# nubot-nudt/LCR-Net

Hardware: AMD Instinct MI355X
Metric: scans/s (120k-pt KITTI-shape scan -> 256-D descriptor) (higher is better)
Workload: dtype f32 (K-deep GEMMs, K >= 288 and N >= 64: fp32 operands as bf16 x 3 split, 6 of 9 products on the bf16 matrix cores, fp32 accumulate — error vs fp64 <= the fp32-MFMA kernel's; every other GEMM, KPConv and attention: fp32 MFMA); 1 GPU; configs[1]: batch of 8 synthetic 64-beam scans (~120k pts, 0.3 m voxel -> ~16k pts), voxelise + 3 subsamples + 10 radius searches + KPConv encoder + NetVLAD, seeded random weights; distinct_input_batches=4, streams=pre-processing stream (own host thread, 2 batches ahead) + 2 encoder stream(s), parallelism=scan-parallel x1, all-gather of descriptors

## Files before the change

include/lcr_hip_debug.h:

```cpp
#ifndef LCR_HIP_DEBUG_H
#define LCR_HIP_DEBUG_H

#ifdef __cplusplus
extern "C" {
#endif

void lcr_gemm_debug_force_tile(int tile);
void lcr_gemm_debug_deep(int mode);
void lcr_gemm_debug_streamk(int mode);
void lcr_groupnorm_debug_general(int on);
void lcr_kpconv_debug_off64(int on);

#ifdef __cplusplus
}
#endif
#endif
```

lcr-net_amd/_lib.py:

```python
import ctypes
import os
import re
import types

import torch

_PKG = os.path.dirname(os.path.abspath(__file__))
LIB_PATH = os.path.join(_PKG, "liblcr_hip.so")

_lib = None

HEADERS = [os.path.join(_PKG, "..", "include", h) for h in ("lcr_hip.h", "lcr_hip_debug.h")]
_SCALARS = {"int": ctypes.c_int, "int64_t": ctypes.c_int64, "uint32_t": ctypes.c_uint32, "uint64_t": ctypes.c_uint64, "unsigned": ctypes.c_uint,
            "size_t": ctypes.c_size_t, "float": ctypes.c_float, "double": ctypes.c_double}
_RESULTS = {"int": ctypes.c_int, "void": None, "const char*": ctypes.c_char_p}


def parse_header(text):
    text = re.sub(r"/\*.*?\*/|//[^\n]*", " ", text, flags=re.S)
    text = re.sub(r"^\s*#.*$", "", text, flags=re.M)
    sigs = {}
    for m in re.finditer(r"\b(lcr_\w+)\s*\(", text):
        name = m.group(1)
        head = text[:m.start()]
        res = re.sub(r"\s*\*", "*", " ".join(head[max(head.rfind(c) for c in ";{}") + 1:].split()))
        tail = re.match(r"([^()]*)\)\s*;", text[m.end():])
        if res not in _RESULTS or tail is None:
            raise RuntimeError("%s: cannot parse its prototype (result type %r)" % (name, res))
        args = []
        for p in ([] if tail.group(1).strip() in ("", "void") else tail.group(1).split(",")):
            words = re.sub(r"\bconst\b", " ", p).split()
            ctype = ctypes.c_void_p if "*" in p else _SCALARS.get(" ".join(words[:-1] if len(words) > 1 else words))
            if ctype is None:
                raise RuntimeError("%s: parameter %r has no ctypes mapping" % (name, " ".join(p.split())))
            args.append(ctype)
        sigs[name] = (_RESULTS[res], args)
    return sigs


_RELEASES_GIL = {"lcr_roformer_forward", "lcr_precompute_batch", "lcr_precompute_batch_rows", "lcr_precompute_batch_rows_ex", "lcr_hashmap_bucket_host", "lcr_encoder_forward", "lcr_encoder_forward_ex", "lcr_ktimer_read",
                 "lcr_ktimer_read2", "lcr_hashmap_order_host", "lcr_ransac_sample_host", "lcr_icp_point_to_point", "lcr_icp_point_to_plane", "lcr_netvlad_forward", "lcr_log_sinkhorn", "lcr_log_sinkhorn_ex",
                 "lcr_local_global_registration", "lcr_local_global_registration_ex", "lcr_retrieval_topk", "lcr_stream_spin"}


def build():
    import importlib.util
    spec = importlib.util.spec_from_file_location("_lcr_build", os.path.join(_PKG, "csrc", "build.py"))
    mod = importlib.util.module_from_spec(spec)
    spec.loader.exec_module(mod)
    return mod.build()


_RETURNS_VALUE = {"lcr_version", "lcr_kpconv_mask_ok", "lcr_gemm_split_ok", "lcr_ktimer_read", "lcr_ktimer_read2"}


def __getattr__(name):
    if name == "call":
        lib()
        return call
    raise AttributeError(name)


def _raise_on_rc(rc, fn, args):
    if rc:
        check(rc, fn.__name__)
    return rc


def lib():
    global _lib, call
    if _lib is None:
        if not os.path.exists(LIB_PATH):
            raise RuntimeError(
                "liblcr_hip.so not found at %s — build it with `python lcr-net_amd/csrc/build.py` "
                "(there is no CPU fallback for the lcr-net_amd hot path)" % LIB_PATH)
        sigs = {}
        for header in HEADERS:
            with open(header) as f:
                sigs.update(parse_header(f.read()))
        L = ctypes.CDLL(LIB_PATH)
        K = ctypes.PyDLL(LIB_PATH) if os.environ.get("LCR_CTYPES_KEEP_GIL", "1") != "0" else L
        checked = types.SimpleNamespace()
        for name, (res, args) in sigs.items():
            if not hasattr(L, name):
                continue
            dll = L if name in _RELEASES_GIL else K
            for view, fn in ((L, getattr(dll, name)), (checked, dll[name])):
                fn.restype, fn.argtypes = res, args
                if view is checked and res is ctypes.c_int and name not in _RETURNS_VALUE:
                    fn.errcheck = _raise_on_rc
                setattr(view, name, fn)
        _lib, call = L, checked
    return _lib


def check(rc, what):
    if rc != 0:
        msg = lib().lcr_last_error()
        raise RuntimeError("%s failed (rc=%d): %s" % (what, rc, msg.decode() if msg else ""))


def ptr(t):
    return ctypes.c_void_p(t.data_ptr()) if t is not None else ctypes.c_void_p(0)


def stream_ptr(device=None):
    idx = device.index if isinstance(device, torch.device) else None
    if idx is None:
        idx = torch.cuda.current_device() if not isinstance(device, int) else device
    return ctypes.c_void_p(torch._C._cuda_getCurrentRawStream(idx))


def require_cuda(*tensors):
    for t in tensors:
        if t is not None and not t.is_cuda:
            raise RuntimeError("lcr-net_amd ops run on the GPU only: got a %s tensor (no CPU fallback)" % t.device)


def workspace(nbytes, device):
    return torch.empty(max(int(nbytes), 256), dtype=torch.uint8, device=device)


def ws_size(name, *args):
    lib()
    n = ctypes.c_size_t(0)
    getattr(call, name)(*args, ctypes.byref(n))
    return n.value


def ws(name, *args, device):
    return workspace(ws_size(name, *args), device)
```

lcr-net_amd/csrc/gemm.h:

```cpp
#pragma once
#include <cstdlib>

#include "common.h"

namespace lcr {

typedef float floatx16 __attribute__((ext_vector_type(16)));

constexpr int GM_BK = 32;
constexpr int GM_T = 256;

constexpr int GM_MAX_BATCH = 64;
struct GemmBatch {
  int     count;
  int     strided;
  int     k[GM_MAX_BATCH];
  int64_t a_off[GM_MAX_BATCH], b_off[GM_MAX_BATCH], c_off[GM_MAX_BATCH];
};

struct GemmEpilogue {
  const float*   bias;
  const float*   rowdiv;
  const int64_t* seg_len;
  int            S;
  int            groups;
  double*        stats;
};

struct ANorm {
  const double* stats;
  const float*  gamma;
  const float*  beta;
  int           groups;
  float         eps, slope;
};
constexpr int AN_KMAX = 256;

__device__ __forceinline__ float4 ld4(const float* p) { return *reinterpret_cast<const float4*>(p); }

__device__ __forceinline__ void anorm_load_affine(const ANorm& an, int K, float (&an_g)[2], float (&an_b)[2]) {
#pragma unroll
  for (int u = 0; u < 2; ++u) {
    const int e = threadIdx.x + u * GM_T;
    an_g[u] = an_b[u] = 0.f;
    if (e < 2 * K) {
      const int k = e >= K ? e - K : e;
      an_g[u] = an.gamma[k];
      an_b[u] = an.beta[k];
    }
  }
}

__device__ __forceinline__ void anorm_build_table(const ANorm& an, const GemmEpilogue& ep, int K, int blk_first, const float (&an_g)[2],
                                                  const float (&an_b)[2], float* __restrict__ s_an) {
  const int gs = K / an.groups;
  __shared__ float2 s_mr[2 * 64];
  for (int e = threadIdx.x; e < 2 * an.groups; e += GM_T) {
    const int slot = e >= an.groups ? 1 : 0, g = e - slot * an.groups;
    const int sg = min(blk_first + slot, ep.S - 1);
    const double cnt = static_cast<double>(ep.seg_len[sg]) * gs;
    double sx = 0.0, sxx = 0.0;
    for (int rep = 0; rep < GN_REPLICAS; ++rep) {
      const int64_t o = ((static_cast<int64_t>(rep) * ep.S + sg) * an.groups + g) * 2;
      sx += an.stats[o];
      sxx += an.stats[o + 1];
    }
    const double mean = sx / cnt;
    const double var = fmax(sxx / cnt - mean * mean, 0.0);
    s_mr[e] = make_float2(static_cast<float>(mean), static_cast<float>(1.0 / sqrt(var + static_cast<double>(an.eps))));
  }
  __syncthreads();
#pragma unroll
  for (int u = 0; u < 2; ++u) {
    const int e = threadIdx.x + u * GM_T;
    if (e < 2 * K) {
      const int slot = e >= K ? 1 : 0, k = e - slot * K;
      const float2 mr = s_mr[slot * an.groups + k / gs];
      const float sc = mr.y * an_g[u];
      s_an[slot * 2 * AN_KMAX + k] = sc;
      s_an[slot * 2 * AN_KMAX + AN_KMAX + k] = fmaf(-mr.x, sc, an_b[u]);
    }
  }
  __syncthreads();
}

template <int BM, int BN, int WM, int WN, int NT>
__device__ __forceinline__ void gemm_epilogue(floatx16 (&acc)[NT], float* __restrict__ C, int64_t M, int N, int64_t m0, int n0, int64_t m_tile,
                                              const GemmEpilogue& ep, const float (&bias_v)[NT], int blk_first, int64_t blk_seg_start,
                                              int64_t blk_seg_end, int wm, int wn, int lane) {
  const bool want_stats = ep.stats != nullptr;
  const int gs = want_stats ? N / ep.groups : 1;
  const int64_t wrow0 = m0 + wm * 32;

  const bool interior = m0 + BM <= M && n0 + BN <= N && M * static_cast<int64_t>(N) < (int64_t(1) << 30);
  if (interior) {
    const unsigned row_l = static_cast<unsigned>(wrow0) + 4u * static_cast<unsigned>(lane >> 5);
#pragma unroll
    for (int j = 0; j < NT; ++j) {
      const unsigned col = static_cast<unsigned>(n0 + wn * (32 * NT) + j * 32 + (lane & 31));
      const float bv = bias_v[j];
      const unsigned off0 = row_l * static_cast<unsigned>(N) + col;
      if (ep.rowdiv) {
#pragma unroll
        for (int r = 0; r < 16; ++r) {
          const unsigned dr = static_cast<unsigned>((r & 3) + 8 * (r >> 2));
          const float v = acc[j][r] / ep.rowdiv[row_l + dr] + bv;
          C[off0 + dr * static_cast<unsigned>(N)] = v;
          acc[j][r] = v;
        }
      } else {
#pragma unroll
        for (int r = 0; r < 16; ++r) {
          const unsigned dr = static_cast<unsigned>((r & 3) + 8 * (r >> 2));
          const float v = acc[j][r] + bv;
          C[off0 + dr * static_cast<unsigned>(N)] = v;
          acc[j][r] = v;
        }
      }
    }
  } else
#pragma unroll
  for (int j = 0; j < NT; ++j) {
    const int col = n0 + wn * (32 * NT) + j * 32 + (lane & 31);
    const float bv = bias_v[j];
#pragma unroll
    for (int r = 0; r < 16; ++r) {
      const int64_t row = wrow0 + (r & 3) + 8 * (r >> 2) + 4 * (lane >> 5);
      float v = acc[j][r];
      if (row < M) {
        if (ep.rowdiv) v = v / ep.rowdiv[row];
        v += bv;
        if (col < N) C[row * N + col] = v;
      } else {
        v = 0.f;
      }
      acc[j][r] = v;
    }
  }

  if (want_stats) {
    __shared__ float s_part[2][2 * WM][BN];
    double* rep = ep.stats + static_cast<int64_t>(m_tile % GN_REPLICAS) * ep.S * ep.groups * 2;
    int64_t seg_start = blk_seg_start, seg_end = blk_seg_end;
    const int64_t blk_last_row = min(m0 + BM - 1, M - 1);
    constexpr int GN_EXACT_ROWS = 32;
    auto exact_segment = [&](int64_t rows) { return rows < GN_EXACT_ROWS && gs <= 32; };
    const bool uniform = blk_last_row < seg_end && !exact_segment(seg_end - seg_start);
    if (uniform) {
#pragma unroll
      for (int j = 0; j < NT; ++j) {
        float s = 0.f, ss = 0.f;
#pragma unroll
        for (int r = 0; r < 16; ++r) {
          s += acc[j][r];
          ss = fmaf(acc[j][r], acc[j][r], ss);
        }
        const int cl = wn * (32 * NT) + j * 32 + (lane & 31);
        s_part[0][2 * wm + (lane >> 5)][cl] = s;
        s_part[1][2 * wm + (lane >> 5)][cl] = ss;
      }
      __syncthreads();
      if (threadIdx.x < BN) {
        const int cl = threadIdx.x;
// ... 98 lines not shown
```

lcr-net_amd/csrc/gemm_f32.hip:

```cpp
#include <cstdio>
#include <map>
#include <mutex>
#include <type_traits>

#include "gemm.h"

namespace lcr {

template <int R, int LD, bool VEC, bool RM = false>
struct LoaderT {
  static constexpr int PIECES = R * 8 / GM_T;
  float4 reg[PIECES];
  unsigned okmask;
  int kb;
  __device__ __forceinline__ void load(const float* __restrict__ src, int64_t rows_total, int K, int64_t r0, int k0) {
    kb = k0;
#pragma unroll
    for (int j = 0; j < PIECES; ++j) {
      const int f = threadIdx.x + GM_T * j;
      const int row = f >> 3, c4 = f & 7;
      int64_t gr = r0 + row;
      gr = gr < rows_total ? gr : rows_total - 1;
      const int gk = k0 + c4 * 4;
      if (VEC) {
// ... 527 lines not shown
static int sk_cu_count() {
  static const int n = [] {
    int dev = 0, cus = 0;
    hipGetDevice(&dev);
    if (hipDeviceGetAttribute(&cus, hipDeviceAttributeMultiprocessorCount, dev) != hipSuccess || cus <= 0) cus = 256;
    return cus;
  }();
  return n;
}

static bool sk_worth(int64_t M, int N, int K) {
  const int cus = sk_cu_count();
  const int64_t tiles = static_cast<int64_t>(div_up(M, 64)) * div_up(N, 64);
  if (K < 480 || tiles < cus / 2 || tiles > 6 * static_cast<int64_t>(cus) || tiles > SK_MAX_TILES) return false;
  const double avg = static_cast<double>(tiles) / cus;
  const double worst = static_cast<double>((tiles + cus - 1) / cus);
  return worst / avg >= 1.10;
}

static int launch_gemm_sk(const float* A, const float* B, float* C, int64_t M, int N, int K, const GemmEpilogue& ep, hipStream_t st) {
  const int cus = sk_cu_count();
  const int64_t iters = static_cast<int64_t>(div_up(M, 64)) * div_up(N, 64) * div_up(K, GM_BK);
  int per_cu = 3;
  while (per_cu > 1 && iters / (static_cast<int64_t>(cus) * per_cu) < 24) --per_cu;
  per_cu = env_int("LCR_SK_PER_CU", per_cu);
  int U = cus * per_cu / 8;
  if (U < 1) U = 1;
  if (8 * U > SK_MAX_GRID) U = SK_MAX_GRID / 8;
  int dev = 0;
  hipGetDevice(&dev);
  GemmStreamK sk;
  {
    std::lock_guard<std::mutex> lk(g_sk_mu);
    SkScratch& sc = g_sk_scratch[{dev, st}];
    if (!sc.partial) {
      if (hipMalloc(reinterpret_cast<void**>(&sc.partial), sizeof(float) * 2 * 16 * GM_T * SK_MAX_GRID) != hipSuccess ||
          hipMalloc(reinterpret_cast<void**>(&sc.arrived), sizeof(uint32_t) * SK_MAX_TILES) != hipSuccess) {
        set_error("lcr_gemm_f32: cannot allocate the stream-K scratch");
        return LCR_EHIP;
      }
      hipMemsetAsync(sc.arrived, 0, sizeof(uint32_t) * SK_MAX_TILES, st);
    }
    sk.partial = sc.partial;
    sk.arrived = sc.arrived;
    sk.U = U;
  }
  LCR_LAUNCH_TIMED((k_gemm_f32_sk<64, 64, 2, 2>), dim3(8 * U), dim3(GM_T), 0, st, A, B, C, M, N, K, ep, sk);
  return check_launch("lcr_gemm_f32");
}

}

using namespace lcr;

static int g_force_tile = 0;
extern "C" void lcr_gemm_debug_force_tile(int t) { g_force_tile = t; }
static int g_force_streamk = -1;
static int g_force_deep = -1;
extern "C" void lcr_gemm_debug_deep(int mode) { g_force_deep = mode; }
extern "C" void lcr_gemm_debug_streamk(int mode) { g_force_streamk = mode; }

enum GemmForm { GF_SCALAR, GF_FORCED_TILE, GF_SHORT, GF_DEEP, GF_STREAMK, GF_TILE };
static GemmForm gemm_form(int64_t M, int N, int K, int transA, int transB, bool vec) {
  static const bool no_short = getenv("LCR_GEMM_NO_SHORT") != nullptr;
  static const int short_k = env_int("LCR_GEMM_SHORT_K", 256);
  static const int deep_env = env_int("LCR_GEMM_DEEP", 1);
  static const int sk_env = env_int("LCR_GEMM_STREAMK", 0);
  if (!vec) return GF_SCALAR;
  if (g_force_tile >= 1 && g_force_tile <= 5) return GF_FORCED_TILE;
  const int deep_mode = g_force_deep >= 0 ? g_force_deep : deep_env;
  const bool deep_ok = !transA && transB && K % GM_BK == 0 && !g_force_tile && M * K < (int64_t(1) << 30) && static_cast<int64_t>(N) * K < (int64_t(1) << 30);
  if (deep_mode == 2 && deep_ok) return GF_DEEP;
  if (!no_short && K <= short_k && !transA) return GF_SHORT;
  if (deep_mode && deep_ok) return GF_DEEP;
  if (N <= 32) return GF_TILE;
  const int sk_mode = g_force_streamk >= 0 ? g_force_streamk : sk_env;
  const bool sk_legal = !transA && !transB && K >= 64 && static_cast<int64_t>(div_up(M, 64)) * div_up(N, 64) <= SK_MAX_TILES;
  if (sk_mode && sk_legal && (sk_mode == 2 || sk_worth(M, N, K))) return GF_STREAMK;
  return GF_TILE;
}

static bool gemm_split_light(int N, int K) {
  switch (K) {
    case 128: return N == 64 || N == 256 || N == 512;
    case 256: return N == 64 || N == 128 || N == 512 || N == 1024;
    default: return false;
  }
}
extern "C" int lcr_gemm_split_ok(int N, int K) {
  static const bool light = env_int("LCR_GEMM_SPLIT_LIGHT", 1) != 0;
  if (N < 64 || K < GM_BK || K % GM_BK != 0) return 0;
  return K >= 288 || (light && K <= AN_KMAX && gemm_split_light(N, K));
}

extern "C" int lcr_gemm_f32_anorm(const float* A, const float* B, float* C, int64_t M, int N, int K, const float* bias,
                                  const double* a_stats, const float* a_gamma, const float* a_beta, int a_groups, float a_eps,
                                  float a_slope, const int64_t* seg_len, int S, int groups, double* stats, void* stream) {
  if (!A || !B || !C || M < 0 || N <= 32 || K <= 0 || K > AN_KMAX || K % 4 != 0 || !a_stats || !a_gamma || !a_beta || a_groups < 1 ||
      K % a_groups != 0 || a_groups > 64 || !seg_len || S < 1 || reinterpret_cast<uintptr_t>(A) % 16 != 0 || reinterpret_cast<uintptr_t>(B) % 16 != 0) {
    set_error("lcr_gemm_f32_anorm: needs 32 < N, K <= 256, K % 4 == 0, a_groups dividing K, a segment table and 16-byte aligned operands");
    return LCR_EARG;
  }
  if (!gemm_stats_ok("lcr_gemm_f32_anorm", stats, seg_len, S, groups, N)) return LCR_EARG;
  hipStream_t st = static_cast<hipStream_t>(stream);
  KernelTimerScope timed(KT_GEMM, st, M, N, K);
  if (M == 0) return LCR_OK;
  GemmEpilogue ep{bias, nullptr, seg_len, S, groups, stats};
  ANorm an{a_stats, a_gamma, a_beta, a_groups, a_eps, a_slope};
  LCR_LAUNCH_TIMED((k_gemm_f32<64, 64, 2, 2, false, true, true, true, true>), dim3(gemm_grid(M, N, 64, 64)), dim3(GM_T), 0, st, A, B, C, M,
                     N, K, ep, GemmBatch{}, an);
  return check_launch("lcr_gemm_f32_anorm");
}

extern "C" int lcr_gemm_f32(const float* A, const float* B, float* C, int64_t M, int N, int K, int transA, int transB, const float* bias,
                            const float* rowdiv, const int64_t* seg_len, int S, int groups, double* stats, void* stream) {
  if (!A || !B || !C || M < 0 || N <= 0 || K <= 0) {
    set_error("lcr_gemm_f32: bad argument");
    return LCR_EARG;
  }
  if (!gemm_stats_ok("lcr_gemm_f32", stats, seg_len, S, groups, N)) return LCR_EARG;
  hipStream_t st = static_cast<hipStream_t>(stream);
  KernelTimerScope timed(KT_GEMM, st, M, N, K);
  if (M == 0) return LCR_OK;
  GemmEpilogue ep{bias, rowdiv, seg_len, S, groups, stats};
  const int64_t lda = transA ? M : K, ldb = transB ? K : N;
  const bool vec = (lda % 4 == 0) && (ldb % 4 == 0) && (reinterpret_cast<uintptr_t>(A) % 16 == 0) && (reinterpret_cast<uintptr_t>(B) % 16 == 0);
  switch (gemm_form(M, N, K, transA, transB, vec)) {
    case GF_SCALAR: return launch_gemm<128, 64, 4, 1, false>(A, B, C, M, N, K, transA, transB, ep, st);
    case GF_FORCED_TILE:
      switch (g_force_tile) {
        case 1: return launch_gemm<128, 128, 4, 1, true>(A, B, C, M, N, K, transA, transB, ep, st);
        case 2: return launch_gemm<128, 64, 4, 1, true>(A, B, C, M, N, K, transA, transB, ep, st);
        case 3: return launch_gemm<128, 32, 4, 1, true>(A, B, C, M, N, K, transA, transB, ep, st);
        case 4: return launch_gemm<64, 64, 2, 2, true>(A, B, C, M, N, K, transA, transB, ep, st);
        default: return launch_gemm<64, 128, 2, 2, true>(A, B, C, M, N, K, transA, transB, ep, st);
      }
    case GF_SHORT:
      if (N <= 32) return launch_gemm<128, 32, 4, 1, true, true>(A, B, C, M, N, K, transA, transB, ep, st);
      return launch_gemm<64, 64, 2, 2, true, true>(A, B, C, M, N, K, transA, transB, ep, st);
    case GF_DEEP: return gemm_deep_launch(A, B, C, M, N, K, ep, st, nullptr, 0);
    case GF_STREAMK: return launch_gemm_sk(A, B, C, M, N, K, ep, st);
    case GF_TILE: break;
  }
  if (N <= 32) return launch_gemm<128, 32, 4, 1, true>(A, B, C, M, N, K, transA, transB, ep, st);
  const int64_t b128 = (M + 127) / 128, nb128 = (N + 127) / 128;
  if (K >= 512 && b128 * nb128 >= 512) return launch_gemm<128, 128, 4, 1, true>(A, B, C, M, N, K, transA, transB, ep, st);
  return launch_gemm<64, 64, 2, 2, true>(A, B, C, M, N, K, transA, transB, ep, st);
}

extern "C" int lcr_kpconv_mask_ok(int64_t M, int N, int K, int split) {
  static const bool off = env_int("LCR_KP_MASK", 1) == 0;
  if (off || M <= 0 || N <= 0 || K % 15 != 0 || mask_kshift(K, K / 15) < 0) return 0;
  if (split) return M * static_cast<int64_t>(K) < (int64_t(1) << 29);
  return gemm_form(M, N, K, 0, 1, true) == GF_DEEP;
}

extern "C" int lcr_gemm_f32_batched_ta(const float* A, const float* B, float* C, int64_t M, int N, int count, const int* k_host,
                                       const int64_t* a_off_host, const int64_t* b_off_host, const int64_t* c_off_host, void* stream) {
  if (!A || !B || !C || M <= 0 || N <= 0 || count < 1 || count > GM_MAX_BATCH || !k_host || !a_off_host || !b_off_host || !c_off_host) {
    set_error("lcr_gemm_f32_batched_ta: bad argument (count <= %d)", GM_MAX_BATCH);
    return LCR_EARG;
  }
  GemmBatch bt = {};
  bt.count = count;
  for (int i = 0; i < count; ++i) {
    bt.k[i] = k_host[i];
// ... 42 lines not shown
```

lcr-net_amd/csrc/gemm_split.hip:

```cpp
#include <type_traits>

#include "gemm.h"

namespace lcr {

typedef __bf16 bf16x8_t __attribute__((ext_vector_type(8)));
typedef __bf16 bf16x2_t __attribute__((ext_vector_type(2)));
typedef float f32x2_t __attribute__((ext_vector_type(2)));
typedef float f32x4_t __attribute__((ext_vector_type(4)));
typedef uint32_t u32x4_t __attribute__((ext_vector_type(4)));

__device__ __forceinline__ uint32_t pk_bf16(float a, float b) {
  f32x2_t v = {a, b};
  return __builtin_bit_cast(uint32_t, __builtin_convertvector(v, bf16x2_t));
}
__device__ __forceinline__ void split2(float x0, float x1, uint32_t& h1, uint32_t& h2, uint32_t& h3) {
  h1 = pk_bf16(x0, x1);
  const float r0 = fsub(x0, __uint_as_float(h1 << 16)), r1 = fsub(x1, __uint_as_float(h1 & 0xffff0000u));
  h2 = pk_bf16(r0, r1);
  const float s0 = fsub(r0, __uint_as_float(h2 << 16)), s1 = fsub(r1, __uint_as_float(h2 & 0xffff0000u));
  h3 = pk_bf16(s0, s1);
}

__global__ __launch_bounds__(256) void k_split_bf16x3(const float* __restrict__ w, int64_t n, uint16_t* __restrict__ planes) {
// ... 137 lines not shown
  if constexpr (ANORM) anorm_load_affine(an, K, an_g, an_b);
  int blk_first = 0;
  int64_t blk_seg_start = 0, blk_seg_end = 0;
  if (ep.stats != nullptr || ANORM) {
    blk_seg_end = ep.seg_len[0];
    while (blk_first + 1 < ep.S && m0 >= blk_seg_end) {
      ++blk_first;
      blk_seg_start = blk_seg_end;
      blk_seg_end += ep.seg_len[blk_first];
    }
  }
  if constexpr (ANORM) {
    const int an_split = static_cast<int>(min(static_cast<int64_t>(BM), blk_seg_end - m0));
#pragma unroll
    for (int j = 0; j < 2; ++j) toff[j] = (srow + j * (T / 8) >= an_split ? 2 * AN_KMAX : 0) + spc * 4;
    anorm_build_table(an, ep, K, blk_first, an_g, an_b, s_an);
  }
  park(I0{}, 0, 0);
  fetch_a(I0{}, 2);
  fetch_b(I1{}, 1);
  __syncthreads();
  auto step = [&](auto lds_c, int t) {
    constexpr int P = decltype(lds_c)::value;
    using NX = std::integral_constant<int, P ^ 1>;
    const char* la = sA + P * STGA + fa;
    bf16x8_t a[4][3];
    auto mm = [&](const bf16x8_t& x, const u32x4_t& y, f32x4_t& c) {
      if constexpr (ABL & 1) {
        asm volatile("" ::"v"(x), "v"(y));
      } else {
        c = __builtin_amdgcn_mfma_f32_16x16x32_bf16(x, __builtin_bit_cast(bf16x8_t, y), c, 0, 0, 0);
      }
    };
    if constexpr (ABL & 16) {
      u32x4_t z = {static_cast<uint32_t>(t), 0u, 0u, 0u};
      asm volatile("" : "+v"(z));
#pragma unroll
      for (int b = 0; b < 4; ++b)
#pragma unroll
        for (int p = 0; p < 3; ++p) a[b][p] = __builtin_bit_cast(bf16x8_t, z);
      (void)la;
    } else {
#pragma unroll
      for (int b = 0; b < 4; ++b)
#pragma unroll
        for (int p = 0; p < 3; ++p) a[b][p] = __builtin_bit_cast(bf16x8_t, *reinterpret_cast<const u32x4_t*>(la + p * PLA + b * (16 * RS)));
    }
    const u32x4_t &b0 = rb[P][0], &b1 = rb[P][1], &b2 = rb[P][2];
    auto six = [&](int b) {
      mm(a[b][2], b0, acc[b]);
      mm(a[b][0], b2, acc2[b]);
      mm(a[b][1], b1, acc[b]);
      mm(a[b][1], b0, acc2[b]);
      mm(a[b][0], b1, acc[b]);
      mm(a[b][0], b0, acc2[b]);
    };
    six(0), six(1);
    park(NX{}, P ^ 1, t + 1);
    six(2), six(3);
    if constexpr (!(ABL & 8)) fetch_a(NX{}, t + 3);
    if constexpr (!(ABL & (8 | 32))) fetch_b(lds_c, t + 2);
    __syncthreads();
  };
  int t = 0;
  for (; t + 2 <= nk; t += 2) {
    step(I0{}, t);
    step(I1{}, t + 1);
  }
  if (t < nk) step(I0{}, t);
  float* sC = reinterpret_cast<float*>(sA);
  static_assert(64 * 65 * 4 <= 2 * STGA, "the output tile fits the A stages");
#pragma unroll
  for (int b = 0; b < 4; ++b)
#pragma unroll
    for (int r = 0; r < 4; ++r) sC[(16 * b + 4 * (lane >> 4) + r) * 65 + 16 * wn + (lane & 15)] = acc[b][r] + acc2[b][r];
  __syncthreads();
  const int wm2 = wn >> 1, wn2 = wn & 1;
  floatx16 accs[1];
#pragma unroll
  for (int r = 0; r < 16; ++r) accs[0][r] = sC[(32 * wm2 + (r & 3) + 8 * (r >> 2) + 4 * (lane >> 5)) * 65 + 32 * wn2 + (lane & 31)];
  gemm_epilogue<BM, BN, 2, 2, 1>(accs, C, M, N, m0, n0, m_tile, ep, bias_v, blk_first, blk_seg_start, blk_seg_end, wm2, wn2, lane);
}

}

using namespace lcr;

extern "C" int lcr_split_bf16x3(const float* w, int64_t n, uint16_t* planes, void* stream) {
  if (!w || !planes || n < 0) {
    set_error("lcr_split_bf16x3: bad argument");
    return LCR_EARG;
  }
  if (n == 0) return LCR_OK;
  hipLaunchKernelGGL(k_split_bf16x3, dim3(min(div_up(n, 512), 2048)), dim3(256), 0, static_cast<hipStream_t>(stream), w, n, planes);
  return check_launch("lcr_split_bf16x3");
}

extern "C" int lcr_split_bf16x3_tiles(const float* w, int N, int K, uint16_t* tiles, void* stream) {
  if (!w || !tiles || N < 1 || K < GM_BK || K % GM_BK != 0 || reinterpret_cast<uintptr_t>(w) % 16 != 0 || reinterpret_cast<uintptr_t>(tiles) % 16 != 0) {
    set_error("lcr_split_bf16x3_tiles: needs K %% 32 == 0 and 16-byte aligned buffers");
    return LCR_EARG;
  }
  hipLaunchKernelGGL(k_split_bf16x3_tiles, dim3(div_up(N, 64) * (K / GM_BK)), dim3(256), 0, static_cast<hipStream_t>(stream), w, N, K, tiles);
  return check_launch("lcr_split_bf16x3_tiles");
}

static int bsplit_impl(const float* A, const uint16_t* Bs, float* C, int64_t M, int N, int K, const float* bias, const float* rowdiv,
                       const int64_t* seg_len, int S, int groups, double* stats, const uint16_t* amask, int kshift, void* stream) {
  if (!A || !Bs || !C || M < 0 || N <= 0 || K <= 0 || K % GM_BK != 0 || reinterpret_cast<uintptr_t>(A) % 16 != 0 || reinterpret_cast<uintptr_t>(Bs) % 16 != 0 ||
      K < GM_BK) {
    set_error("lcr_gemm_f32_bsplit: needs K %% 32 == 0 and 16-byte aligned operands");
    return LCR_EARG;
  }
  if (!gemm_stats_ok("lcr_gemm_f32_bsplit", stats, seg_len, S, groups, N)) return LCR_EARG;
  hipStream_t st = static_cast<hipStream_t>(stream);
  KernelTimerScope timed(KT_GEMM, st, M, N, K);
  if (M == 0) return LCR_OK;
  GemmEpilogue ep{bias, rowdiv, seg_len, S, groups, stats};
  static const int abl = env_int("LCR_SPLIT_ABL", 0);
  const dim3 grid(gemm_grid(M, N, 64, 64)), block(256);
  if (amask) {
    LCR_LAUNCH_TIMED((k_gemm_f32_bsplit_p<0, true>), grid, block, 0, st, A, Bs, C, M, N, K, ep, amask, kshift, ANorm{});
    return check_launch("lcr_gemm_f32_bsplit_masked");
  }
  switch (abl) {
    case 1: LCR_LAUNCH_TIMED((k_gemm_f32_bsplit_p<1>), grid, block, 0, st, A, Bs, C, M, N, K, ep, amask, kshift, ANorm{}); break;
    case 2: LCR_LAUNCH_TIMED((k_gemm_f32_bsplit_p<2>), grid, block, 0, st, A, Bs, C, M, N, K, ep, amask, kshift, ANorm{}); break;
    case 4: LCR_LAUNCH_TIMED((k_gemm_f32_bsplit_p<4>), grid, block, 0, st, A, Bs, C, M, N, K, ep, amask, kshift, ANorm{}); break;
    case 8: LCR_LAUNCH_TIMED((k_gemm_f32_bsplit_p<8>), grid, block, 0, st, A, Bs, C, M, N, K, ep, amask, kshift, ANorm{}); break;
    case 16: LCR_LAUNCH_TIMED((k_gemm_f32_bsplit_p<16>), grid, block, 0, st, A, Bs, C, M, N, K, ep, amask, kshift, ANorm{}); break;
    case 23: LCR_LAUNCH_TIMED((k_gemm_f32_bsplit_p<23>), grid, block, 0, st, A, Bs, C, M, N, K, ep, amask, kshift, ANorm{}); break;
    case 30: LCR_LAUNCH_TIMED((k_gemm_f32_bsplit_p<30>), grid, block, 0, st, A, Bs, C, M, N, K, ep, amask, kshift, ANorm{}); break;
    case 32: LCR_LAUNCH_TIMED((k_gemm_f32_bsplit_p<32>), grid, block, 0, st, A, Bs, C, M, N, K, ep, amask, kshift, ANorm{}); break;
    default: LCR_LAUNCH_TIMED((k_gemm_f32_bsplit_p<0>), grid, block, 0, st, A, Bs, C, M, N, K, ep, amask, kshift, ANorm{}); break;
  }
  return check_launch("lcr_gemm_f32_bsplit");
}

extern "C" int lcr_gemm_f32_bsplit(const float* A, const uint16_t* Bs, float* C, int64_t M, int N, int K, const float* bias, const float* rowdiv,
                                   const int64_t* seg_len, int S, int groups, double* stats, void* stream) {
  return bsplit_impl(A, Bs, C, M, N, K, bias, rowdiv, seg_len, S, groups, stats, nullptr, 0, stream);
}

extern "C" int lcr_gemm_f32_bsplit_anorm(const float* A, const uint16_t* Bs, float* C, int64_t M, int N, int K, const float* bias,
                                         const double* a_stats, const float* a_gamma, const float* a_beta, int a_groups, float a_eps,
                                         float a_slope, const int64_t* seg_len, int S, int groups, double* stats, void* stream) {
  if (!A || !Bs || !C || M < 0 || N < 64 || K < GM_BK || K > AN_KMAX || K % GM_BK != 0 || !a_stats || !a_gamma || !a_beta || a_groups < 1 ||
      K % a_groups != 0 || a_groups > 64 || !seg_len || S < 1 || reinterpret_cast<uintptr_t>(A) % 16 != 0 || reinterpret_cast<uintptr_t>(Bs) % 16 != 0) {
    set_error("lcr_gemm_f32_bsplit_anorm: needs N >= 64, K <= 256, K %% 32 == 0, a_groups (<= 64) dividing K, a segment table and 16-byte aligned operands");
    return LCR_EARG;
  }
  if (!gemm_stats_ok("lcr_gemm_f32_bsplit_anorm", stats, seg_len, S, groups, N)) return LCR_EARG;
  hipStream_t st = static_cast<hipStream_t>(stream);
  KernelTimerScope timed(KT_GEMM, st, M, N, K);
  if (M == 0) return LCR_OK;
  GemmEpilogue ep{bias, nullptr, seg_len, S, groups, stats};
  ANorm an{a_stats, a_gamma, a_beta, a_groups, a_eps, a_slope};
  LCR_LAUNCH_TIMED((k_gemm_f32_bsplit_p<0, false, true>), dim3(gemm_grid(M, N, 64, 64)), dim3(256), 0, st, A, Bs, C, M, N, K, ep,
                   static_cast<const uint16_t*>(nullptr), 0, an);
  return check_launch("lcr_gemm_f32_bsplit_anorm");
}

extern "C" int lcr_gemm_f32_bsplit_masked(const float* A, const uint16_t* Bs, float* C, int64_t M, int N, int K, const float* bias,
                                          const float* rowdiv, const int64_t* seg_len, int S, int groups, double* stats, const uint16_t* row_mask,
                                          int block_k, void* stream) {
  const int ks = mask_kshift(K, block_k);
  if (!row_mask || ks < 0 || M * static_cast<int64_t>(K) >= (int64_t(1) << 29)) {
    set_error("lcr_gemm_f32_bsplit_masked: needs a row mask, block_k = 32 << s (s <= 3) with K <= 16 block_k, and M*K < 2^29");
    return LCR_EARG;
  }
  return bsplit_impl(A, Bs, C, M, N, K, bias, rowdiv, seg_len, S, groups, stats, row_mask, ks, stream);
}
```

lcr-net_amd/functional.py:

```python
import ctypes
import os
import threading

import numpy as np
import torch

from . import _lib

GN_EPS = 1e-5
GN_REPLICAS = 8


class KernelTimer:
    KINDS = {"gemm": 0, "kpconv_aggregate": 1, "radius_query": 2, "attention": 3, "kpconv_fused": 4, "sinkhorn": 5}

    def __init__(self, names):
        self.names = set(names)
        self._cache = None

    def summary(self):
        return {k: [(b, m) for b, _, m in v] for k, v in self.records().items()}

    def records(self):
        if self._cache is None:
# ... 64 lines not shown
        _ARENA.off = 0
        return self

    def __exit__(self, *exc):
        _ARENA.buf, _ARENA.off = self.prev
        return False


def _zero_stats(S, groups, device):
    n = GN_REPLICAS * S * groups * 2
    buf = _ARENA.buf
    if buf is not None and buf.device == device and _ARENA.off + n <= buf.numel():
        v = buf[_ARENA.off:_ARENA.off + n].view(GN_REPLICAS, S, groups, 2)
        _ARENA.off += n
        return v
    return torch.zeros((GN_REPLICAS, S, groups, 2), dtype=torch.float64, device=device)


def _gemm_out(M, N, seg_len, groups, device, always_seg=False):
    c = torch.empty((M, N), dtype=torch.float32, device=device)
    if not (groups or always_seg):
        return c, None, 0, None
    if seg_len is None:
        seg_len = torch.full((1,), int(M), dtype=torch.int64, device=device)
    S = seg_len.numel()
    return c, seg_len, S, (_zero_stats(S, groups, device) if groups else None)


def gemm(a, b, trans_b=False, trans_a=False, bias=None, rowdiv=None, seg_len=None, groups=0, row_mask=None):
    if row_mask is not None:
        return _gemm_masked(a, b, trans_b, trans_a, bias, rowdiv, seg_len, groups, row_mask)
    _lib.require_cuda(a, b)
    assert a.dtype == torch.float32 and b.dtype == torch.float32 and a.is_contiguous() and b.is_contiguous()
    M, K = (a.shape[1], a.shape[0]) if trans_a else (a.shape[0], a.shape[1])
    N = b.shape[0] if trans_b else b.shape[1]
    assert (b.shape[1] if trans_b else b.shape[0]) == K, "inner dimensions differ"
    c, seg_len, S, stats = _gemm_out(M, N, seg_len, groups, a.device)
    _lib.call.lcr_gemm_f32(
        _lib.ptr(a), _lib.ptr(b), _lib.ptr(c), M, N, K, int(trans_a), int(trans_b), _lib.ptr(bias), _lib.ptr(rowdiv),
        _lib.ptr(seg_len), S, int(groups), _lib.ptr(stats), _lib.stream_ptr(a.device))
    return c, stats


def kpconv_mask_ok(M, N, K, split):
    return bool(_lib.lib().lcr_kpconv_mask_ok(int(M), int(N), int(K), int(bool(split))))


def _mask_args(a, row_mask):
    M, K = a.shape
    assert row_mask.dtype == torch.int16 and row_mask.is_contiguous() and row_mask.numel() == M and row_mask.device == a.device
    assert K % 15 == 0
    return K // 15


def _gemm_masked(a, b, trans_b, trans_a, bias, rowdiv, seg_len, groups, row_mask):
    _lib.require_cuda(a, b)
    assert trans_b and not trans_a, "the masked form takes A [M,K] and B [N,K]"
    assert a.dtype == torch.float32 and b.dtype == torch.float32 and a.is_contiguous() and b.is_contiguous()
    block_k = _mask_args(a, row_mask)
    M, K = a.shape
    N = b.shape[0]
    assert b.shape[1] == K, "inner dimensions differ"
    c, seg_len, S, stats = _gemm_out(M, N, seg_len, groups, a.device)
    _lib.call.lcr_gemm_f32_masked(
        _lib.ptr(a), _lib.ptr(b), _lib.ptr(c), M, N, K, _lib.ptr(bias), _lib.ptr(rowdiv), _lib.ptr(seg_len), S,
        int(groups), _lib.ptr(stats), _lib.ptr(row_mask), block_k, _lib.stream_ptr(a.device))
    return c, stats


_GEMM_SPLIT = [os.environ.get("LCR_GEMM_SPLIT", "1") not in ("", "0")]


def gemm_split_enabled():
    return _GEMM_SPLIT[0]


def set_gemm_split(on):
    _GEMM_SPLIT[0] = bool(on)


_GEMM_SPLIT_LIGHT = os.environ.get("LCR_GEMM_SPLIT_LIGHT", "1") not in ("", "0")


_GEMM_SPLIT_LIGHT_CLASSES = {(64, 128), (256, 128), (512, 128), (64, 256), (128, 256), (512, 256), (1024, 256)}


def _gemm_split_light(N, K):
    return (N, K) in _GEMM_SPLIT_LIGHT_CLASSES


def gemm_split_ok(N, K):
    if N < 64 or K < 32 or K % 32 != 0:
        return False
    return K >= 288 or (_GEMM_SPLIT_LIGHT and K <= ANORM_MAX_K and _gemm_split_light(N, K))


derived_lock = threading.RLock()


class WeightStamp:
    __slots__ = ("ref", "ptr", "ver", "dev")

    def __init__(self, t):
        import weakref
        self.ref, self.ptr, self.ver, self.dev = weakref.ref(t), t.data_ptr(), t._version, t.device

    def same(self, t):
        return self.ref is not None and self.ref() is t and self.ptr == t.data_ptr() and self.ver == t._version and self.dev == t.device

    def __reduce__(self):
        return (_dead_stamp, ())


def _dead_stamp():
    s = WeightStamp.__new__(WeightStamp)
    s.ref, s.ptr, s.ver, s.dev = None, 0, -1, None
    return s


def drop_derived(module, *names):
    for n in names:
        if n in module.__dict__:
            module.__dict__[n] = None



def publish_derived(t):
    torch.cuda.current_stream(t.device).synchronize()
    return t


def split_bf16x3(w):
    w = w.detach().contiguous()
    N, K = w.shape
    assert K % 32 == 0
    tiles = torch.empty(((N + 63) // 64, K // 32, 3, 64, 32), dtype=torch.int16, device=w.device)
    _lib.call.lcr_split_bf16x3_tiles(_lib.ptr(w), int(N), int(K), _lib.ptr(tiles), _lib.stream_ptr(w.device))
    tiles.lcr_n = int(N)
    return tiles


def unsplit_bf16x3(tiles, padded=False):
    CT, KS = tiles.shape[0], tiles.shape[1]
    t = tiles.view(CT, KS, 4, 3, 4, 16, 8)
    t = t.permute(3, 0, 2, 5, 1, 4, 6).reshape(3, CT * 64, KS * 32)
    if not padded:
        t = t[:, :tiles.lcr_n]
    return t.contiguous().view(torch.bfloat16).float()


def gemm_bsplit(a, planes, bias=None, rowdiv=None, seg_len=None, groups=0, row_mask=None):
    _lib.require_cuda(a, planes)
    assert a.dtype == torch.float32 and a.is_contiguous() and planes.dtype == torch.int16 and planes.is_contiguous() and planes.dim() == 5
    M, K = a.shape
    N = planes.lcr_n
    assert planes.shape[1] * 32 == K and planes.shape[0] == (N + 63) // 64, "inner dimensions differ"
    c, seg_len, S, stats = _gemm_out(M, N, seg_len, groups, a.device)
    if row_mask is not None:
        block_k = _mask_args(a, row_mask)
        _lib.call.lcr_gemm_f32_bsplit_masked(_lib.ptr(a), _lib.ptr(planes), _lib.ptr(c), M, N, K, _lib.ptr(bias), _lib.ptr(rowdiv), _lib.ptr(seg_len),
                                             S, int(groups), _lib.ptr(stats), _lib.ptr(row_mask), block_k, _lib.stream_ptr(a.device))
        return c, stats
    _lib.call.lcr_gemm_f32_bsplit(_lib.ptr(a), _lib.ptr(planes), _lib.ptr(c), M, N, K, _lib.ptr(bias), _lib.ptr(rowdiv),
                                  _lib.ptr(seg_len), S, int(groups), _lib.ptr(stats), _lib.stream_ptr(a.device))
    return c, stats


# ... 1472 lines not shown
```

Baseline: 3157 scans/s.

## Add short-K bf16x3 split GEMM kernel reusing A tile across column tiles

Adds a specialized bf16x3 split GEMM kernel for K of 32 or 64. It loads and splits (and optionally group-normalizes) the A tile once, then loops over one or more 64-column output tiles, prefetching the next B tile. It also routes the (N=128, K=32/64) GEMM shapes onto the split path instead of plain fp32 MFMA, and adds debug hooks to force the column-tile count. The aim is to cut per-tile A reload and normalization overhead for shallow GEMMs, at the cost of fewer workgroups when ct>1 and a new code path to validate.

```diff
diff --git a/include/lcr_hip_debug.h b/include/lcr_hip_debug.h
--- a/include/lcr_hip_debug.h
+++ b/include/lcr_hip_debug.h
@@ -8,6 +8,8 @@
 void lcr_gemm_debug_force_tile(int tile);
 void lcr_gemm_debug_deep(int mode);
 void lcr_gemm_debug_streamk(int mode);
+void lcr_gemm_debug_split_shortk(int mode);
+int lcr_gemm_debug_split_last_ct(void);
 void lcr_groupnorm_debug_general(int on);
 void lcr_kpconv_debug_off64(int on);
 
diff --git a/lcr-net_amd/_lib.py b/lcr-net_amd/_lib.py
--- a/lcr-net_amd/_lib.py
+++ b/lcr-net_amd/_lib.py
@@ -51,7 +51,7 @@
     return mod.build()
 
 
-_RETURNS_VALUE = {"lcr_version", "lcr_kpconv_mask_ok", "lcr_gemm_split_ok", "lcr_ktimer_read", "lcr_ktimer_read2"}
+_RETURNS_VALUE = {"lcr_version", "lcr_kpconv_mask_ok", "lcr_gemm_split_ok", "lcr_ktimer_read", "lcr_ktimer_read2", "lcr_gemm_debug_split_last_ct"}
 
 
 def __getattr__(name):
diff --git a/lcr-net_amd/csrc/gemm.h b/lcr-net_amd/csrc/gemm.h
--- a/lcr-net_amd/csrc/gemm.h
+++ b/lcr-net_amd/csrc/gemm.h
@@ -51,6 +51,7 @@
   }
 }
 
+template <int KS = AN_KMAX>
 __device__ __forceinline__ void anorm_build_table(const ANorm& an, const GemmEpilogue& ep, int K, int blk_first, const float (&an_g)[2],
                                                   const float (&an_b)[2], float* __restrict__ s_an) {
   const int gs = K / an.groups;
@@ -77,8 +78,8 @@
       const int slot = e >= K ? 1 : 0, k = e - slot * K;
       const float2 mr = s_mr[slot * an.groups + k / gs];
       const float sc = mr.y * an_g[u];
-      s_an[slot * 2 * AN_KMAX + k] = sc;
-      s_an[slot * 2 * AN_KMAX + AN_KMAX + k] = fmaf(-mr.x, sc, an_b[u]);
+      s_an[slot * 2 * KS + k] = sc;
+      s_an[slot * 2 * KS + KS + k] = fmaf(-mr.x, sc, an_b[u]);
     }
   }
   __syncthreads();
diff --git a/lcr-net_amd/csrc/gemm_f32.hip b/lcr-net_amd/csrc/gemm_f32.hip
--- a/lcr-net_amd/csrc/gemm_f32.hip
+++ b/lcr-net_amd/csrc/gemm_f32.hip
@@ -633,6 +633,8 @@
 
 static bool gemm_split_light(int N, int K) {
   switch (K) {
+    case 32: return N == 128;
+    case 64: return N == 128;
     case 128: return N == 64 || N == 256 || N == 512;
     case 256: return N == 64 || N == 128 || N == 512 || N == 1024;
     default: return false;
diff --git a/lcr-net_amd/csrc/gemm_split.hip b/lcr-net_amd/csrc/gemm_split.hip
--- a/lcr-net_amd/csrc/gemm_split.hip
+++ b/lcr-net_amd/csrc/gemm_split.hip
@@ -243,9 +243,190 @@
   gemm_epilogue<BM, BN, 2, 2, 1>(accs, C, M, N, m0, n0, m_tile, ep, bias_v, blk_first, blk_seg_start, blk_seg_end, wm2, wn2, lane);
 }
 
+template <int NK, bool ANORM>
+__global__ __launch_bounds__(256, 4) void k_gemm_f32_bsplit_wk(const float* __restrict__ A, const uint16_t* __restrict__ Bs, float* __restrict__ C, int64_t M,
+                                                             int N, GemmEpilogue ep, int ct, ANorm an) {
+  constexpr int BM = 64, BN = 64, RS = 64, T = 256, PLA = BM * RS, K = NK * GM_BK;
+  constexpr bool HALF = NK == 2;
+  __shared__ __attribute__((aligned(16))) char sA[NK * 3 * PLA];
+  __shared__ float sC[(HALF ? 32 : 64) * 65];
+  const int lane = threadIdx.x & 63, wn = __builtin_amdgcn_readfirstlane(threadIdx.x >> 6);
+  const int ntn = (N + BN - 1) / BN, ncg = (ntn + ct - 1) / ct;
+  const int xcd = blockIdx.x & 7, slot = blockIdx.x >> 3;
+  const int64_t m_tile = static_cast<int64_t>(slot / ncg) * 8 + xcd;
+  const int64_t m0 = m_tile * BM;
+  const int ct0 = (slot % ncg) * ct, ct1 = min(ct0 + ct, ntn);
+  if (m0 >= M) return;
+  const int srow = threadIdx.x >> 3, spc = threadIdx.x & 7;
+  f32x4_t ra[NK][2];
+  int soff[2];
+#pragma unroll
+  for (int j = 0; j < 2; ++j) {
+    const int r = srow + j * (T / 8);
+    int64_t ga = m0 + r;
+    ga = ga < M ? ga : M - 1;
+    const float* ap = A + ga * K + spc * 4;
+#pragma unroll
+    for (int ks = 0; ks < NK; ++ks) ra[ks][j] = *reinterpret_cast<const f32x4_t*>(ap + ks * GM_BK);
+    soff[j] = r * RS + (((spc >> 1) ^ ((r >> 2) & 3)) << 4) + (spc & 1) * 8;
+  }
+  const char* bp = reinterpret_cast<const char*>(Bs) + wn * 3072 + lane * 16;
+  u32x4_t rb[NK][3], rbn[NK][3];
+  float bias_v[1], bias_n;
+  auto fetch_b = [&](int c) {
+    const char* p0 = bp + static_cast<int64_t>(c) * (NK * 12288);
+#pragma unroll
+    for (int ks = 0; ks < NK; ++ks)
+#pragma unroll
+      for (int p = 0; p < 3; ++p) rbn[ks][p] = *reinterpret_cast<const u32x4_t*>(p0 + ks * 12288 + p * 1024);
+    const int col = c * BN + (wn & 1) * 32 + (lane & 31);
+    bias_n = (ep.bias && col < N) ? ep.bias[col] : 0.f;
+  };
+  fetch_b(ct0);
+  __shared__ __attribute__((aligned(16))) float s_an[ANORM ? 4 * K : 4];
+  float an_g[2], an_b[2];
+  if constexpr (ANORM) anorm_load_affine(an, K, an_g, an_b);
+  int blk_first = 0;
+  int64_t blk_seg_start = 0, blk_seg_end = 0;
+  if (ep.stats != nullptr || ANORM) {
+    blk_seg_end = ep.seg_len[0];
+    while (blk_first + 1 < ep.S && m0 >= blk_seg_end) {
+      ++blk_first;
+      blk_seg_start = blk_seg_end;
+      blk_seg_end += ep.seg_len[blk_first];
+    }
+  }
+  int toff[2] = {0, 0};
+  if constexpr (ANORM) {
+    const int an_split = static_cast<int>(min(static_cast<int64_t>(BM), blk_seg_end - m0));
+#pragma unroll
+    for (int j = 0; j < 2; ++j) toff[j] = (srow + j * (T / 8) >= an_split ? 2 * K : 0) + spc * 4;
+    anorm_build_table<K>(an, ep, K, blk_first, an_g, an_b, s_an);
+  }
+#pragma unroll
+  for (int ks = 0; ks < NK; ++ks)
+#pragma unroll
+    for (int j = 0; j < 2; ++j) {
+      f32x4_t v = ra[ks][j];
+      if constexpr (ANORM) {
+        const float* tb = s_an + toff[j] + ks * GM_BK;
+        const float4 sc = *reinterpret_cast<const float4*>(tb), sh = *reinterpret_cast<const float4*>(tb + K);
+        v.x = fmaf(v.x, sc.x, sh.x), v.y = fmaf(v.y, sc.y, sh.y), v.z = fmaf(v.z, sc.z, sh.z), v.w = fmaf(v.w, sc.w, sh.w);
+        v.x = v.x > 0.f ? v.x : v.x * an.slope, v.y = v.y > 0.f ? v.y : v.y * an.slope;
+        v.z = v.z > 0.f ? v.z : v.z * an.slope, v.w = v.w > 0.f ? v.w : v.w * an.slope;
+      }
+      uint32_t h1, h2, h3, g1, g2, g3;
+      split2(v.x, v.y, h1, h2, h3);
+      split2(v.z, v.w, g1, g2, g3);
+      char* da = sA + ks * (3 * PLA) + soff[j];
+      *reinterpret_cast<uint2*>(da) = make_uint2(h1, g1);
+      *reinterpret_cast<uint2*>(da + PLA) = make_uint2(h2, g2);
+      *reinterpret_cast<uint2*>(da + 2 * PLA) = make_uint2(h3, g3);
+    }
+  __syncthreads();
+  const int fa = (lane & 15) * RS + (((lane >> 4) ^ (((lane & 15) >> 2) & 3)) << 4);
+  const int wm2 = wn >> 1, wn2 = wn & 1;
+  for (int c = ct0; c < ct1; ++c) {
+    int lane_e = lane;
+    asm volatile("" : "+v"(lane_e));
+#pragma unroll
+    for (int ks = 0; ks < NK; ++ks)
+#pragma unroll
+      for (int p = 0; p < 3; ++p) rb[ks][p] = rbn[ks][p];
+    bias_v[0] = bias_n;
+    if (c + 1 < ct1) fetch_b(c + 1);
+    f32x4_t acc[4], acc2[4];
+#pragma unroll
+    for (int b = 0; b < 4; ++b) acc[b] = acc2[b] = f32x4_t{0.f, 0.f, 0.f, 0.f};
+#pragma unroll
+    for (int ks = 0; ks < NK; ++ks) {
+      const char* la = sA + ks * (3 * PLA) + fa;
+      auto mm = [&](const bf16x8_t& x, const u32x4_t& y, f32x4_t& d) {
+        d = __builtin_amdgcn_mfma_f32_16x16x32_bf16(x, __builtin_bit_cast(bf16x8_t, y), d, 0, 0, 0);
+      };
+      const u32x4_t &b0 = rb[ks][0], &b1 = rb[ks][1], &b2 = rb[ks][2];
+#pragma unroll
+      for (int h = 0; h < 2; ++h) {
+        bf16x8_t a[2][3];
+#pragma unroll
+        for (int b = 0; b < 2; ++b)
+#pragma unroll
+          for (int p = 0; p < 3; ++p) a[b][p] = __builtin_bit_cast(bf16x8_t, *reinterpret_cast<const u32x4_t*>(la + p * PLA + (2 * h + b) * (16 * RS)));
+#pragma unroll
+        for (int b = 0; b < 2; ++b) {
+          mm(a[b][2], b0, acc[2 * h + b]);
+          mm(a[b][0], b2, acc2[2 * h + b]);
+          mm(a[b][1], b1, acc[2 * h + b]);
+          mm(a[b][1], b0, acc2[2 * h + b]);
+          mm(a[b][0], b1, acc[2 * h + b]);
+          mm(a[b][0], b0, acc2[2 * h + b]);
+        }
+        __builtin_amdgcn_sched_barrier(0);
+      }
+    }
+    floatx16 accs[1];
+    if constexpr (HALF) {
+#pragma unroll
+      for (int h = 0; h < 2; ++h) {
+        if (h) __syncthreads();
+#pragma unroll
+        for (int b = 0; b < 2; ++b)
+#pragma unroll
+          for (int r = 0; r < 4; ++r) sC[(16 * b + 4 * (lane >> 4) + r) * 65 + 16 * wn + (lane & 15)] = acc[2 * h + b][r] + acc2[2 * h + b][r];
+        __syncthreads();
+        if (wm2 == h)
+#pragma unroll
+          for (int r = 0; r < 16; ++r) accs[0][r] = sC[((r & 3) + 8 * (r >> 2) + 4 * (lane_e >> 5)) * 65 + 32 * wn2 + (lane_e & 31)];
+      }
+    } else {
+#pragma unroll
+      for (int b = 0; b < 4; ++b)
+#pragma unroll
+        for (int r = 0; r < 4; ++r) sC[(16 * b + 4 * (lane >> 4) + r) * 65 + 16 * wn + (lane & 15)] = acc[b][r] + acc2[b][r];
+      __syncthreads();
+#pragma unroll
+      for (int r = 0; r < 16; ++r) accs[0][r] = sC[(32 * wm2 + (r & 3) + 8 * (r >> 2) + 4 * (lane_e >> 5)) * 65 + 32 * wn2 + (lane_e & 31)];
+    }
+#pragma unroll
+    for (int ks = 0; ks < NK; ++ks)
+#pragma unroll
+      for (int p = 0; p < 3; ++p) asm volatile("" ::"v"(rbn[ks][p]));
+    asm volatile("" ::"v"(bias_n) : "memory");
+    gemm_epilogue<BM, BN, 2, 2, 1>(accs, C, M, N, m0, c * BN, m_tile, ep, bias_v, blk_first, blk_seg_start, blk_seg_end, wm2, wn2, lane_e);
+    if (c + 1 < ct1) __syncthreads();
+  }
+}
+
 }
 
 using namespace lcr;
+
+static int g_force_shortk = -1;
+static int g_split_last_ct = 0;
+extern "C" void lcr_gemm_debug_split_shortk(int mode) { g_force_shortk = mode; }
+extern "C" int lcr_gemm_debug_split_last_ct(void) { return g_split_last_ct; }
+
+constexpr int SHORTK_MIN_WORKGROUPS = 1536;
+static int bsplit_shortk_ct(int64_t M, int N, int K, bool anorm) {
+  static const int env = env_int("LCR_SPLIT_SHORTK", 1);
+  const int mode = g_force_shortk >= 0 ? g_force_shortk : env;
+  if (mode == 0 || K > 2 * GM_BK) return 0;
+  const int ntn = div_up(N, 64);
+  if (mode == 2) return ntn;
+  if (mode == 3) return 1;
+  if (mode == 4) return min(2, ntn);
+  return (anorm && ntn >= 2 && static_cast<int64_t>(div_up(M, 64)) * div_up(ntn, 2) >= SHORTK_MIN_WORKGROUPS) ? 2 : 1;
+}
+
+template <bool ANORM>
+static void bsplit_shortk_launch(const float* A, const uint16_t* Bs, float* C, int64_t M, int N, int K, const GemmEpilogue& ep, const ANorm& an, int ct,
+                                 hipStream_t st) {
+  const dim3 grid((div_up(M, 64) + 7) / 8 * 8 * div_up(div_up(N, 64), ct)), block(256);
+  if (K == GM_BK)
+    LCR_LAUNCH_TIMED((k_gemm_f32_bsplit_wk<1, ANORM>), grid, block, 0, st, A, Bs, C, M, N, ep, ct, an);
+  else
+    LCR_LAUNCH_TIMED((k_gemm_f32_bsplit_wk<2, ANORM>), grid, block, 0, st, A, Bs, C, M, N, ep, ct, an);
+}
 
 extern "C" int lcr_split_bf16x3(const float* w, int64_t n, uint16_t* planes, void* stream) {
   if (!w || !planes || n < 0) {
@@ -280,6 +461,12 @@
   GemmEpilogue ep{bias, rowdiv, seg_len, S, groups, stats};
   static const int abl = env_int("LCR_SPLIT_ABL", 0);
   const dim3 grid(gemm_grid(M, N, 64, 64)), block(256);
+  g_split_last_ct = 0;
+  if (const int ct = (amask || abl) ? 0 : bsplit_shortk_ct(M, N, K, false)) {
+    g_split_last_ct = ct;
+    bsplit_shortk_launch<false>(A, Bs, C, M, N, K, ep, ANorm{}, ct, st);
+    return check_launch("lcr_gemm_f32_bsplit");
+  }
   if (amask) {
     LCR_LAUNCH_TIMED((k_gemm_f32_bsplit_p<0, true>), grid, block, 0, st, A, Bs, C, M, N, K, ep, amask, kshift, ANorm{});
     return check_launch("lcr_gemm_f32_bsplit_masked");
@@ -317,6 +504,11 @@
   if (M == 0) return LCR_OK;
   GemmEpilogue ep{bias, nullptr, seg_len, S, groups, stats};
   ANorm an{a_stats, a_gamma, a_beta, a_groups, a_eps, a_slope};
+  g_split_last_ct = bsplit_shortk_ct(M, N, K, true);
+  if (g_split_last_ct) {
+    bsplit_shortk_launch<true>(A, Bs, C, M, N, K, ep, an, g_split_last_ct, st);
+    return check_launch("lcr_gemm_f32_bsplit_anorm");
+  }
   LCR_LAUNCH_TIMED((k_gemm_f32_bsplit_p<0, false, true>), dim3(gemm_grid(M, N, 64, 64)), dim3(256), 0, st, A, Bs, C, M, N, K, ep,
                    static_cast<const uint16_t*>(nullptr), 0, an);
   return check_launch("lcr_gemm_f32_bsplit_anorm");
diff --git a/lcr-net_amd/functional.py b/lcr-net_amd/functional.py
--- a/lcr-net_amd/functional.py
+++ b/lcr-net_amd/functional.py
@@ -170,7 +170,8 @@
 _GEMM_SPLIT_LIGHT = os.environ.get("LCR_GEMM_SPLIT_LIGHT", "1") not in ("", "0")
 
 
-_GEMM_SPLIT_LIGHT_CLASSES = {(64, 128), (256, 128), (512, 128), (64, 256), (128, 256), (512, 256), (1024, 256)}
+_GEMM_SPLIT_LIGHT_CLASSES = {(64, 128), (256, 128), (512, 128), (64, 256), (128, 256), (512, 256), (1024, 256),
+                             (128, 32), (128, 64)}
 
 
 def _gemm_split_light(N, K):
```

Result: slower. 3087 scans/s (-2.2%).
